# Ecogenomics/CheckM

Hardware: NVIDIA H100
Metric: genomes/hour (higher is better)
Workload: dtype int16 (SSV) / u8 (MSV) / int16 (Viterbi) / f32 (Forward, domain definition)

## Files before the change

checkm_b200/csrc/fwdback_blk.cuh:

```cuda
#pragma once
#include "device_utils.cuh"
#include "engine.hpp"
#include "fwdback.cuh"

namespace ckm {

constexpr int BLK_LOOKAHEAD_MAXQ = 16;

template <int Q, bool TSMEM>
struct BlkModel {
  int M;
  const float *rfb;
  const float4 *tsm;
  float4 t0[TSMEM ? 1 : Q], t1[TSMEM ? 1 : Q];
  int lane;
  __device__ __forceinline__ float4 T0(int q) const { return TSMEM ? tsm[q * 32 + lane] : t0[TSMEM ? 0 : q]; }
  __device__ __forceinline__ float4 T1(int q) const { return TSMEM ? tsm[(Q + q) * 32 + lane] : t1[TSMEM ? 0 : q]; }
};

template <int Q, bool TSMEM>
__device__ __forceinline__ void blk_model_load(BlkModel<Q, TSMEM> &bm, const ModelScalars &ms, const float4 *tfb, const float *rfb,
                                               float4 *tsm, int lane) {
  bm.M = ms.M; bm.lane = lane;
  bm.rfb = rfb + ms.blk_off * 32 * KPAD + lane;
  bm.tsm = tsm;
  const float4 *src = tfb + ms.blk_off * 32 * 2;
  if (TSMEM) {
    __syncwarp();
    for (int q = 0; q < Q; ++q) { tsm[q * 32 + lane] = __ldg(src + (q * 32 + lane) * 2); tsm[(Q + q) * 32 + lane] = __ldg(src + (q * 32 + lane) * 2 + 1); }
    __syncwarp();
  } else {
#pragma unroll
    for (int q = 0; q < Q; ++q) { bm.t0[TSMEM ? 0 : q] = __ldg(src + (q * 32 + lane) * 2); bm.t1[TSMEM ? 0 : q] = __ldg(src + (q * 32 + lane) * 2 + 1); }
  }
}

template <int Q, bool TSMEM, bool FULL, bool STORE_D = true>
__device__ __forceinline__ float forward_blk(const BlkModel<Q, TSMEM> &bm, const uint8_t *__restrict__ res, int L, const Specials sp,
                                             float *xmx, float *full) {
  const int lane = bm.lane;
  float Mx[Q], Ix[Q], Dx[Q];
#pragma unroll
  for (int q = 0; q < Q; ++q) { Mx[q] = 0.0f; Ix[q] = 0.0f; Dx[q] = 0.0f; }
  if (FULL) {
#pragma unroll
    for (int z = 0; z < 3 * Q; ++z) full[z * 32 + lane] = 0.0f;
  }
  float xE = 0.0f, xN = 1.0f, xJ = 0.0f, xB = sp.nmove, xC = 0.0f, totscale = 0.0f;
  if (xmx != nullptr && lane == 0) { xmx[X_E] = xE; xmx[X_N] = xN; xmx[X_J] = xJ; xmx[X_B] = xB; xmx[X_C] = xC; xmx[X_SCALE] = 1.0f; }
  constexpr bool LA = (Q <= BLK_LOOKAHEAD_MAXQ);
  float ecur[Q];
  int xnext;
  if (LA) {
    const float *rp = bm.rfb + (size_t)((L >= 1) ? __ldg(res) : 0) * Q * 32;
#pragma unroll
    for (int q = 0; q < Q; ++q) ecur[q] = __ldg(rp + q * 32);
    xnext = (L >= 2) ? __ldg(res + 1) : 0;
  } else xnext = (L >= 1) ? __ldg(res) : 0;
// ... 209 lines not shown
```

checkm_b200/csrc/kernels_blk.cu:

```cuda
#include "engine.hpp"
#include "device_utils.cuh"
#include "stages.hpp"
#include "fwdback.cuh"
#include "fwdback_blk.cuh"
#include "domdef_common.cuh"

namespace ckm {

constexpr int BLK_WARPS = 4;

template <int Q> __host__ __device__ constexpr size_t blk_tsm_bytes() { return (size_t)Q * 32 * 2 * sizeof(float4); }

template <int Q, bool TSMEM>
__global__ void __launch_bounds__(BLK_WARPS * 32) fwd2_kernel(FilterParams p) {
  extern __shared__ __align__(16) uint8_t bsm[];
  const int lane = threadIdx.x & 31, warp = threadIdx.x >> 5;
  float4 *tsm = reinterpret_cast<float4 *>(bsm) + (size_t)warp * Q * 32 * 2;
  const int n = min(*p.in_count, p.in_cap);
  for (int c = blockIdx.x * BLK_WARPS + warp; c < n; c += gridDim.x * BLK_WARPS) {
    Candidate cd = p.in[c];
    const ModelScalars ms = p.ms[cd.model];
    if (ms.vq != Q) continue;
    const int s = cd.seq, L = p.len[s];
    BlkModel<Q, TSMEM> bm;
    blk_model_load<Q, TSMEM>(bm, ms, p.tfb, p.rfb, tsm, lane);
    const float fsc = forward_blk<Q, TSMEM, false>(bm, p.res + p.off[s], L, make_specials(L, true), nullptr, nullptr);
    cd.fwdsc = fsc;
    const float seq_score = __fdiv_rn(__fsub_rn(fsc, cd.filtersc), 0.69314718055994529f);
    const double P = exp_surv((double)seq_score, (double)ms.evparam[4], (double)ms.evparam[5]);
    cd.P = P;
    if (lane == 0) {
      if (p.dense_fwd != nullptr) p.dense_fwd[(int64_t)p.model_slot[cd.model] * p.nseq + s] = fsc;
      if (P <= p.F3) {
        const int pos = atomicAdd(p.out_count, 1);
        if (pos < p.out_cap) p.out[pos] = cd;
        if (p.dense_passed != nullptr) atomicOr_u8(p.dense_passed, (int64_t)p.model_slot[cd.model] * p.nseq + s, 8);
      }
    }
  }
}

template <int Q, bool TSMEM>
__global__ void __launch_bounds__(BLK_WARPS * 32) regions2_kernel(DomdefParams p) {
  extern __shared__ __align__(16) uint8_t bsm[];
  const int lane = threadIdx.x & 31, warp = threadIdx.x >> 5;
  float4 *tsm = reinterpret_cast<float4 *>(bsm) + (size_t)warp * Q * 32 * 2;
  for (int idx = p.pair_begin + blockIdx.x * BLK_WARPS + warp; idx < p.pair_end; idx += gridDim.x * BLK_WARPS) {
    const int pi = p.pair_order[idx];
    const PairWork pw = p.pairs[pi];
    const ModelScalars ms = p.ms[pw.model];
    if (ms.vq != Q) continue;
    const int L = pw.L;
    BlkModel<Q, TSMEM> bm;
    blk_model_load<Q, TSMEM>(bm, ms, p.tfb, p.rfb, tsm, lane);
    const uint8_t *res = p.res + p.off[pw.seq];
    const Specials sp = make_specials(L, true);
    float *xf = p.xf + pw.row_off * X_NX, *xb = p.xb + pw.row_off * X_NX;
    forward_blk<Q, TSMEM, false>(bm, res, L, sp, xf, nullptr);
    __syncwarp();
    backward_blk<Q, TSMEM, 0>(bm, res, L, sp, xf, xb, nullptr);
    __syncwarp();
    regions_tail(p, pi, L, sp, xf, xb, p.btot + pw.row_off, p.etot + pw.row_off, p.mocc + pw.row_off, p.n2sc + pw.row_off, lane);
    __syncwarp();
  }
}

template <int Q, bool TSMEM>
__global__ void __launch_bounds__(BLK_WARPS * 32) envelope2_kernel(DomdefParams p) {
  extern __shared__ __align__(16) uint8_t bsm[];
  const int lane = threadIdx.x & 31, warp = threadIdx.x >> 5;
  float4 *tsm = reinterpret_cast<float4 *>(bsm) + (size_t)warp * Q * 32 * 2;
  float *null2 = reinterpret_cast<float *>(bsm + (TSMEM ? BLK_WARPS * blk_tsm_bytes<Q>() : 0)) + warp * 32;
  constexpr int QW = Q * 32;
  for (int idx = p.env_begin + blockIdx.x * BLK_WARPS + warp; idx < p.env_end; idx += gridDim.x * BLK_WARPS) {
    const int ei = p.env_order[idx];
    const Envelope env = p.envs[ei];
    const PairWork pw = p.pairs[env.pair];
    const ModelScalars ms = p.ms[pw.model];
    if (ms.vq != Q) continue;
    BlkModel<Q, TSMEM> bm;
    blk_model_load<Q, TSMEM>(bm, ms, p.tfb, p.rfb, tsm, lane);
    const int M = ms.M, Ld = env.j - env.i + 1;
    const uint8_t *res = p.res + p.off[pw.seq] + (env.i - 1);
    const Specials sp = make_specials(pw.L, false);
    const int64_t mat = (int64_t)(Ld + 1) * 3 * QW;
    float *F = p.scratch + env.scratch_off, *Bm = F;
    float *xf = F + mat, *xb = xf + (int64_t)(Ld + 1) * X_NX, *pps = xb + (int64_t)(Ld + 1) * X_NX;
    float *xo = xf;
    float *n2sc = p.n2sc + pw.row_off;
    const float envsc = forward_blk<Q, TSMEM, true, false>(bm, res, Ld, sp, xf, F);
    __syncwarp();
    backward_blk<Q, TSMEM, 2>(bm, res, Ld, sp, xf, xb, F);
    __syncwarp();
    const float scaleproduct = __fdiv_rn(1.0f, xb[X_N]);
    float em[Q], ein[Q];
#pragma unroll
    for (int q = 0; q < Q; ++q) { em[q] = 0.0f; ein[q] = 0.0f; }
    for (int r = 1; r <= Ld; ++r) {
      if (r + 2 <= Ld && lane < Q) {
        const float *fn = F + (int64_t)(r + 2) * 3 * QW;
        prefetch_l2(fn + lane * 32); prefetch_l2(fn + (2 * Q + lane) * 32);
      }
      const float totr = scaleproduct * xf[(int64_t)r * X_NX + X_SCALE];
      const float *fr = F + (int64_t)r * 3 * QW + lane;
      float vm[Q], vi[Q];
#pragma unroll
      for (int q = 0; q < Q; ++q) { vm[q] = fr[q * 32]; vi[q] = fr[(2 * Q + q) * 32]; }
#pragma unroll
      for (int q = 0; q < Q; ++q) {
        const float pm = vm[q] * totr, pi = vi[q] * totr;
        em[q] = (r == 1) ? pm : em[q] + pm;
        ein[q] = (r == 1) ? pi : ein[q] + pi;
      }
    }
// ... 192 lines not shown
          s1 = (t1s * xc[X_N] > t1s * xc[X_J]) ? ST_N : ST_J;
        } else { ok = false; break; }
        if (s1 == ST_M) {
          if (!have_last || s0 == ST_E) { lastMi = i; lastMk = k; have_last = true; }
          firstMi = i; firstMk = k;
          if (p.trace != nullptr && lane == 0) p.trace[pw.row_off + env.i - 1 + i] = k;
        } else if (s1 == ST_I) {
          if (p.trace != nullptr && lane == 0) p.trace[pw.row_off + env.i - 1 + i] = -k;
        }
        if ((s1 == ST_N || s1 == ST_J || s1 == ST_C) && s1 == s0) i--;
        s0 = s1;
      }
      if (!have_last) ok = false;
      hmmfrom = firstMk; hmmto = lastMk; sqfrom = firstMi + env.i - 1; sqto = lastMi + env.i - 1;
    }
#undef CELL
#undef TT0
#undef TT1
    if (lane == 0) {
      DomainOut out;
      out.pair = env.pair; out.ienv = env.i; out.jenv = env.j;
      float domcorrection = 0.0f;
      for (int pos = env.i; pos <= env.j; ++pos) domcorrection += n2sc[pos];
      out.ok = ok ? 1 : 0;
      out.envsc = envsc; out.oasc = oasc; out.domcorrection = domcorrection;
      out.hmmfrom = hmmfrom; out.hmmto = hmmto; out.sqfrom = sqfrom; out.sqto = sqto;
      out.bitscore = 0.f; out.dombias = 0.f; out.pad = 0.f; out.lnP = 0.0;
      p.doms[env.slot] = out;
    }
    __syncwarp();
  }
}

template <int Q, bool TSMEM, class P, class KF>
static int launch_one(KF kern, const P &p, int grid, size_t extra, cudaStream_t st, const char *what) {
  const size_t smem = (TSMEM ? BLK_WARPS * blk_tsm_bytes<Q>() : 0) + extra;
  if (smem > 48 * 1024) {
    cudaError_t e = cudaFuncSetAttribute(kern, cudaFuncAttributeMaxDynamicSharedMemorySize, (int)smem);
    if (e != cudaSuccess) return cuda_fail(e, what);
  }
  kern<<<grid, BLK_WARPS * 32, smem, st>>>(p);
  cudaError_t e = cudaGetLastError();
  return e == cudaSuccess ? CKM_OK : cuda_fail(e, what);
}

#define CKM_CLASS_SWITCH(KERN, EXTRA, WHAT)                                                              \
  switch (cls) {                                                                                        \
    case 0: return launch_one<2, false>(KERN<2, false>, p, grid, EXTRA, st, WHAT);                      \
    case 1: return launch_one<4, false>(KERN<4, false>, p, grid, EXTRA, st, WHAT);                      \
    case 2: return launch_one<6, false>(KERN<6, false>, p, grid, EXTRA, st, WHAT);                      \
    case 3: return launch_one<8, false>(KERN<8, false>, p, grid, EXTRA, st, WHAT);                      \
    case 4: return launch_one<12, true>(KERN<12, true>, p, grid, EXTRA, st, WHAT);                      \
    case 5: return launch_one<16, true>(KERN<16, true>, p, grid, EXTRA, st, WHAT);                      \
    case 6: return launch_one<20, true>(KERN<20, true>, p, grid, EXTRA, st, WHAT);                      \
    case 7: return launch_one<24, true>(KERN<24, true>, p, grid, EXTRA, st, WHAT);                      \
    case 8: return launch_one<28, true>(KERN<28, true>, p, grid, EXTRA, st, WHAT);                      \
    case 9: return launch_one<32, true>(KERN<32, true>, p, grid, EXTRA, st, WHAT);                      \
  }                                                                                                     \
  set_error(WHAT ": bad class"); return CKM_EINVAL;

int launch_fwd2(const FilterParams &p, int cls, int grid, cudaStream_t st) { CKM_CLASS_SWITCH(fwd2_kernel, 0, "fwd2_kernel") }
int launch_regions2(const DomdefParams &p, int cls, int grid, cudaStream_t st) { CKM_CLASS_SWITCH(regions2_kernel, 0, "regions2_kernel") }
int launch_envelopes2(const DomdefParams &p, int cls, int grid, cudaStream_t st) {
  const size_t extra = BLK_WARPS * 32 * sizeof(float);
  CKM_CLASS_SWITCH(envelope2_kernel, extra, "envelope2_kernel")
}

}
```

checkm_b200/csrc/search.cu:

```cuda
#include <algorithm>
#include <atomic>
#include <chrono>
#include <cstdio>
#include <cmath>
#include <cstdlib>
#include <cstring>
#include <memory>
#include <vector>
#include "engine.hpp"
#include "stages.hpp"
#include "pool.hpp"

using namespace ckm;

namespace ckm {

std::atomic<int> g_live_engines{0};
thread_local ckm_engine *g_pool_engine = nullptr;
thread_local int g_pool_next = 0;
constexpr int X_NX_HOST = 6;
struct EnsembleJob;
int ensembles_launch(ckm_engine *e, const ckm_models *m, DomdefParams &p, const std::vector<PairWork> &pairs,
                     const std::vector<Region> &regs, const std::vector<int> &multi_idx, const std::vector<EnsembleCaps> &caps,
                     cudaStream_t st, EnsembleJob **job_out);
int ensembles_collect(EnsembleJob *job, cudaStream_t st, std::vector<std::vector<Envelope>> &out, std::vector<EnsembleCaps> &grow, int *n_over);
void ensembles_abandon(EnsembleJob *job, cudaStream_t st);
enum { CTR_UNIT4 = 0, CTR_UNIT8, CTR_UNIT16, CTR_UNIT32, CTR_CAND, CTR_MSV, CTR_BIAS, CTR_VIT, CTR_FWD, CTR_ENV, CTR_DOM, CTR_VREDO, CTR_SSVRES, CTR_VWORK = 16 , CTR_N = 32 };
enum { EV_SSV = 0, EV_MSV, EV_BIAS, EV_VIT, EV_FWD, EV_CASCADE_END, EV_DOMDEF, EV_END, EV_CALL };

static int64_t env_scratch_budget() {
  if (const char *v = std::getenv("CKM_ENV_SCRATCH_MB")) {
    char *end = nullptr;
    const long long mb = std::strtoll(v, &end, 10);
    if (end != v && *end == '\0' && mb > 0) return (int64_t)std::min<long long>(mb, (long long)1 << 30) * ((int64_t)1 << 20) / (int64_t)sizeof(float);
  }
  size_t free_b = 0, total_b = 0;
  cudaMemGetInfo(&free_b, &total_b);
  const size_t neng = (size_t)std::max(1, g_live_engines.load());
  return (int64_t)std::min<size_t>(total_b * 4 / 10 / neng, (size_t)56 << 30) / (int64_t)sizeof(float);
}
struct SearchKnobs { bool blk, vitp, ssv_resolve, trace; int ens_first; int64_t env_budget; };
static SearchKnobs read_knobs(bool envelopes) {
  auto starts = [](const char *name, char c) { const char *v = std::getenv(name); return v != nullptr && v[0] == c; };
  SearchKnobs k;
  k.blk = !starts("CKM_BLK", '0');
  k.vitp = k.blk && !starts("CKM_VITP", '0');
  k.ssv_resolve = !starts("CKM_SSV_RESOLVE", '0');
  k.trace = starts("CKM_TRACE", '1');
  const char *ens = std::getenv("CKM_ENS_FIRST");
  k.ens_first = ens == nullptr ? -1 : (ens[0] == '0' ? 0 : 1);
  k.env_budget = envelopes ? env_scratch_budget() : 0;
  return k;
}
struct Trace {
  bool on; std::chrono::steady_clock::time_point t0, last;
  explicit Trace(bool on_) : on(on_) { t0 = last = std::chrono::steady_clock::now(); }
  void mark(const char *what) {
    if (!on) return;
    const auto now = std::chrono::steady_clock::now();
    std::fprintf(stderr, "[ckm trace] %-28s +%8.3f ms  (%9.3f)\n", what, std::chrono::duration<double, std::milli>(now - last).count(),
                 std::chrono::duration<double, std::milli>(now - t0).count());
    last = now;
  }
};

static int vq_of(int M) { return (M <= 64) ? 2 : (M <= 128) ? 4 : (M <= 192) ? 6 : (M <= 256) ? 8 : (M <= 384) ? 12 : (M <= 512) ? 16 : (M <= 640) ? 20 : (M <= 768) ? 24 : (M <= 896) ? 28 : (M <= 1024) ? 32 : 0; }
static int cls_of(int M, bool use_blk) {
  if (!use_blk) return N_BLK_CLASSES;
  const int q = vq_of(M);
  for (int c = 0; c < N_BLK_CLASSES; ++c) if (BLK_Q[c] == q) return c;
  return N_BLK_CLASSES;
}

static int fan_out(ckm_engine *e) {
  CKM_CUDA(cudaEventRecord(e->fan_ev, e->stream));
  for (auto &s : e->cls) CKM_CUDA(cudaStreamWaitEvent(s, e->fan_ev, 0));
  return CKM_OK;
}
static int fan_in(ckm_engine *e) {
// ... 1 lines not shown
    CKM_CUDA(cudaEventRecord(e->cls_ev[c], e->cls[c]));
    CKM_CUDA(cudaStreamWaitEvent(e->stream, e->cls_ev[c], 0));
  }
  return CKM_OK;
}

template <class P> static int per_class(ckm_engine *e, const P &p, int (*blocked)(const P &, int, int, cudaStream_t), int blk_per_sm,
                                        int (*unblocked)(const P &, int, cudaStream_t), int per_sm, bool widest_first = false) {
  const int nsm = e->prop.multiProcessorCount;
  int rc;
  if ((rc = fan_out(e))) return rc;
  for (int i = 0; i < ckm_engine::NCLS; ++i) {
    const int c = widest_first ? ckm_engine::NCLS - 1 - i : i;
    if (c == N_BLK_CLASSES) rc = unblocked ? unblocked(p, nsm * per_sm, e->cls[c]) : CKM_OK;
    else rc = p.use_blk ? blocked(p, c, nsm * blk_per_sm, e->cls[c]) : CKM_OK;
    if (rc) return rc;
  }
  return fan_in(e);
}
template <class Launch> static int launch_class_runs(ckm_engine *e, const std::vector<int32_t> &order, const std::vector<int8_t> &cls, size_t b0, size_t b1, Launch launch) {
  const int nsm = e->prop.multiProcessorCount;
  int rc;
  if ((rc = fan_out(e))) return rc;
  while (b0 < b1) {
    size_t r1 = b0; const int c = cls[order[b0]];
    while (r1 < b1 && cls[order[r1]] == c) ++r1;
    const int cnt = (int)(r1 - b0);
    const int grid = c < N_BLK_CLASSES ? std::min(nsm * 8, (cnt + 3) / 4) : std::min(nsm * 4, (cnt + FWD_WARPS - 1) / FWD_WARPS);
    if ((rc = launch(c, (int32_t)b0, (int32_t)r1, grid, e->cls[c]))) return rc;
    e->stats.kernel_launches++;
    b0 = r1;
  }
  return CKM_OK;
}

struct ActiveMasks { DevBuf tile_active, model_active, model_slot; bool all_active = true; };
static FilterParams filter_params(const ckm_models *m, const ckm_seqdb *db, ActiveMasks &am) {
  FilterParams p{};
  p.res = db->d_res; p.off = db->d_off; p.len = db->d_len; p.lenA = db->d_lenA; p.lenB = db->d_lenB; p.tmove_w = db->d_tmove_w;
  p.ms = m->d_scalars; p.bias_eo = m->d_bias_eo; p.rwv = m->d_rwv; p.twv = m->d_twv; p.rfv = m->d_rfv; p.tfv = m->d_tfv;
  p.twb = m->d_twb; p.rwb = m->d_rwb; p.tfb = m->d_tfb; p.rfb = m->d_rfb; p.twp = m->d_twp; p.rwp = m->d_rwp;
  p.row_elems = ((m->maxM + 31) / 32) * 32 + 64;
  p.F1 = 0.02; p.F2 = 1e-3; p.F3 = 1e-5;
  p.model_slot = am.model_slot.as<int32_t>(); p.nseq = db->nseq;
  return p;
}

static DomdefParams domdef_params(const ckm_models *m, const ckm_seqdb *db, const SearchKnobs &k) {
  DomdefParams p{};
  p.res = db->d_res; p.off = db->d_off; p.nullsc = db->d_nullsc; p.ms = m->d_scalars; p.rfv = m->d_rfv; p.tfv = m->d_tfv;
  p.row_elems = ((m->maxM + 31) / 32) * 32 + 64;
  p.tfb = m->d_tfb; p.rfb = m->d_rfb; p.use_blk = k.blk ? 1 : 0;
  return p;
}
static void fill_filter_stats(ckm_engine *e, int64_t n_pairs, const int32_t *ctr, unsigned long long cells, int stages) {
  ckm_stats &s = e->stats;
  s.n_pairs = n_pairs; s.n_cells = (int64_t)cells;
  s.n_ssv_cand = (int64_t)ctr[CTR_CAND] + ctr[CTR_SSVRES]; s.n_msv_exact = ctr[CTR_CAND]; s.n_past_msv = ctr[CTR_MSV]; s.n_past_bias = ctr[CTR_BIAS];
  s.n_past_vit = ctr[CTR_VIT]; s.n_past_fwd = ctr[CTR_FWD]; s.n_vit_redo = ctr[CTR_VREDO];
  float *ms[] = {&s.ms_ssv, &s.ms_msv, &s.ms_bias, &s.ms_vit, &s.ms_fwd};
  for (int i = 0; i < stages; ++i) cudaEventElapsedTime(ms[i], e->ev[EV_SSV + i], e->ev[EV_SSV + i + 1]);
}
static std::vector<float> &logsum_table() {
  static std::vector<float> t = [] {
    std::vector<float> v(16000);
    for (int i = 0; i < 16000; ++i) v[i] = (float)std::log(1.0 + std::exp((double)-i / 1000.0));
    return v;
  }();
  return t;
}

static int build_masks(const ckm_models *m, const ckm_seqdb *db, const int32_t *model_idx, int32_t nmodels,
                       const int64_t *bin_model_offsets, ActiveMasks &am, std::vector<int32_t> &slot_of_model, cudaStream_t st) {
  const int ndb = (int)m->models.size(), nbins = db->nbins, ntiles = (int)m->tiles.size();
  slot_of_model.assign(ndb, -1);
  bool all = (bin_model_offsets == nullptr) && (model_idx == nullptr || nmodels == ndb);
  if (model_idx == nullptr) { for (int i = 0; i < ndb; ++i) slot_of_model[i] = i; }
  else if (bin_model_offsets == nullptr) {
    for (int i = 0; i < nmodels; ++i) {
      if (model_idx[i] < 0 || model_idx[i] >= ndb) { set_error("model index out of range"); return CKM_EINVAL; }
      if (slot_of_model[model_idx[i]] >= 0) { set_error("duplicate model index in query list"); return CKM_EINVAL; }
      slot_of_model[model_idx[i]] = i;
    }
    if (all) for (int i = 0; i < ndb; ++i) if (slot_of_model[i] < 0) all = false;
  }
// ... 150 lines not shown
  if ((rc = launch_bias(p, nsm * 8, st))) return rc;
  CKM_CUDA(cudaEventRecord(e->ev[EV_VIT], st));
  p.in = s2.a.as<Candidate>(); p.in_count = e->d_counters + CTR_BIAS; p.in_cap = s2.cap;
  p.out = s2.b.as<Candidate>(); p.out_count = e->d_counters + CTR_VIT; p.out_cap = s2.cap;
  if ((rc = run_viterbi(e, p, k.vitp))) return rc;
  CKM_CUDA(cudaEventRecord(e->ev[EV_FWD], st));
  p.in = s2.b.as<Candidate>(); p.in_count = e->d_counters + CTR_VIT; p.in_cap = s2.cap;
  p.out = s2.a.as<Candidate>(); p.out_count = e->d_counters + CTR_FWD; p.out_cap = s2.cap;
  if ((rc = per_class(e, p, launch_fwd2, 8, launch_fwd, 4, true))) return rc;
  CKM_CUDA(cudaEventRecord(e->ev[EV_CASCADE_END], st));
  e->stats.kernel_launches += 3 + (k.vitp ? N_BLK_CLASSES : 0) + (p.use_blk ? 2 * N_BLK_CLASSES : 0);
  return CKM_OK;
}

static int64_t envelope_need(const ckm_models *m, const PairWork &pw, const Envelope &en, bool use_blk) {
  const int64_t Ld = en.j - en.i + 1, Mpad = ((m->models[pw.model].M + 1) + 31) / 32 * 32 + 32;
  const int64_t vq = use_blk ? vq_of(m->models[pw.model].M) : 0;
  const int64_t width = vq ? 32 * vq : Mpad;
  return (vq ? 1 : 2) * (Ld + 1) * 3 * width + (Ld + 1) * 15 + 64;
}
static int run_envelope_waves(ckm_engine *e, const ckm_models *m, const std::vector<PairWork> &pairs, DomdefParams &p, int64_t budget,
                              DevBuf &scratch, std::vector<Envelope> &ev, DevBuf &d_ev, DevBuf &d_ord, bool leave_last) {
  if (ev.empty()) return CKM_OK;
  cudaStream_t st = e->stream;
  int rc;
  std::vector<int64_t> need(ev.size());
  std::vector<int8_t> ecls(ev.size());
  for (size_t i = 0; i < ev.size(); ++i) {
    const PairWork &pw = pairs[ev[i].pair];
    need[i] = envelope_need(m, pw, ev[i], p.use_blk != 0);
    ecls[i] = (int8_t)cls_of(m->models[pw.model].M, p.use_blk != 0);
  }
  budget = std::max<int64_t>(budget, *std::max_element(need.begin(), need.end()));
  if ((rc = d_ev.alloc(sizeof(Envelope) * ev.size())) || (rc = d_ord.alloc(sizeof(int32_t) * ev.size()))) return rc;
  std::vector<int32_t> eorder(ev.size());
  for (size_t w0 = 0, w1; w0 < ev.size(); w0 = w1) {
    int64_t tot = 0;
    for (w1 = w0; w1 < ev.size() && (w1 == w0 || tot + need[w1] <= budget); ++w1) { ev[w1].scratch_off = tot; tot += need[w1]; }
    if (sizeof(float) * (size_t)tot > scratch.bytes && (rc = scratch.alloc(sizeof(float) * (size_t)tot))) return rc;
    for (size_t i = w0; i < w1; ++i) eorder[i] = (int32_t)i;
    std::stable_sort(eorder.begin() + w0, eorder.begin() + w1, [&](int32_t a, int32_t b) { return ecls[a] != ecls[b] ? ecls[a] > ecls[b] : need[a] > need[b]; });
    CKM_CUDA(cudaMemcpyAsync(d_ev.as<Envelope>() + w0, ev.data() + w0, sizeof(Envelope) * (w1 - w0), cudaMemcpyHostToDevice, st));
    CKM_CUDA(cudaMemcpyAsync(d_ord.as<int32_t>() + w0, eorder.data() + w0, sizeof(int32_t) * (w1 - w0), cudaMemcpyHostToDevice, st));
    p.envs = d_ev.as<Envelope>(); p.env_order = d_ord.as<int32_t>(); p.scratch = scratch.as<float>();
    if ((rc = launch_class_runs(e, eorder, ecls, w0, w1, [&](int c, int32_t b0, int32_t b1, int grid, cudaStream_t s) -> int {
          p.env_begin = b0; p.env_end = b1; return c < N_BLK_CLASSES ? launch_envelopes2(p, c, grid, s) : launch_envelopes(p, grid, s); }))) return rc;
    CKM_CUDA(cudaStreamSynchronize(st));
    if (w1 < ev.size() || !leave_last) { if ((rc = fan_in(e))) return rc; CKM_CUDA(cudaStreamSynchronize(st)); }
  }
  return CKM_OK;
}

struct QueryPlan { ActiveMasks am; bool per_bin = false; std::vector<std::vector<int32_t>> qorder; int64_t n_pairs = 0; };
static int plan_queries(const ckm_models *m, const ckm_seqdb *db, const int32_t *model_idx, int32_t nmodels, const int64_t *bin_model_offsets, QueryPlan &q, cudaStream_t st) {
  const int ndb = (int)m->models.size();
  if (model_idx == nullptr && bin_model_offsets == nullptr) nmodels = ndb;
  std::vector<int32_t> slot;
  int rc = build_masks(m, db, model_idx, nmodels, bin_model_offsets, q.am, slot, st);
  if (rc) return rc;
  q.per_bin = bin_model_offsets != nullptr;
  if (q.per_bin) {
    q.qorder.assign(db->nbins, std::vector<int32_t>(ndb, -1));
    for (int b = 0; b < db->nbins; ++b) {
      for (int64_t i = bin_model_offsets[b]; i < bin_model_offsets[b + 1]; ++i) q.qorder[b][model_idx[i]] = (int32_t)(i - bin_model_offsets[b]);
      q.n_pairs += (int64_t)db->bin_nseq[b] * (bin_model_offsets[b + 1] - bin_model_offsets[b]);
    }
  } else {
    q.qorder.emplace_back(std::move(slot));
    q.n_pairs = (int64_t)db->nseq * nmodels;
  }
  return CKM_OK;
}

static int run_cascade(ckm_engine *e, const SearchKnobs &k, const ckm_models *m, const ckm_seqdb *db, ActiveMasks &am, int64_t n_pairs, Stage1 &s1, Stage2 &s2, int32_t *ctr) {
  cudaStream_t st = e->stream;
  unsigned long long cells = 0;
  int rc;
  for (int attempt = 0; attempt < QUEUE_ATTEMPTS; ++attempt) {
    if (attempt > 0) e->stats.n_queue_retries++;
// ... 23 lines not shown
    pw.first_dom = 0; pw.ndom_slots = 0; pw.fwdsc = fl[i].fwdsc; pw.filtersc = fl[i].filtersc; pw.usc = fl[i].usc;
    pw.row_off = rows; rows += pw.L + 1;
  }
  return CKM_OK;
}
struct DomainStage {
  DomdefParams p{};
  DevBuf dpairs, dxf, dxb, dvec, dtbl, dregions, dporder, ddoms, dhits, dscratch, denvs, deorder, denvs2, deorder2;
  std::vector<Region> regs;
  std::vector<DomainOut> doms; std::vector<HitOut> hout;
};
static int run_regions(ckm_engine *e, const SearchKnobs &k, const ckm_models *m, const ckm_seqdb *db, const std::vector<PairWork> &pairs, int64_t rows, DomainStage &D, Trace &tr) {
  cudaStream_t st = e->stream;
  const int npairs = (int)pairs.size();
  const size_t rws = (size_t)std::max<int64_t>(rows, 1);
  int rc;
  if ((rc = D.dpairs.alloc(sizeof(PairWork) * pairs.size())) || (rc = D.dxf.alloc(sizeof(float) * rws * X_NX_HOST)) || (rc = D.dxb.alloc(sizeof(float) * rws * X_NX_HOST)) ||
      (rc = D.dvec.alloc(sizeof(float) * rws * 4)) || (rc = D.dtbl.alloc(sizeof(float) * 16000))) return rc;
  const int region_cap = npairs * 8 + 1024;
  if ((rc = D.dregions.alloc(sizeof(Region) * (size_t)region_cap))) return rc;
  CKM_CUDA(cudaMemcpyAsync(D.dpairs.p, pairs.data(), sizeof(PairWork) * pairs.size(), cudaMemcpyHostToDevice, st));
  CKM_CUDA(cudaMemcpyAsync(D.dtbl.p, logsum_table().data(), sizeof(float) * 16000, cudaMemcpyHostToDevice, st));
  CKM_CUDA(cudaMemsetAsync(e->d_counters + CTR_ENV, 0, sizeof(int32_t), st));
  DomdefParams &p = D.p = domdef_params(m, db, k);
  p.pairs = D.dpairs.as<PairWork>(); p.npairs = npairs;
  p.xf = D.dxf.as<float>(); p.xb = D.dxb.as<float>();
  p.btot = D.dvec.as<float>(); p.etot = p.btot + rws; p.mocc = p.etot + rws; p.n2sc = p.mocc + rws;
  p.regions = D.dregions.as<Region>(); p.region_count = e->d_counters + CTR_ENV; p.region_cap = region_cap;
  p.logsum_tbl = D.dtbl.as<float>();
  std::vector<int32_t> order((size_t)npairs);
  std::vector<int8_t> pcls((size_t)npairs);
  for (int i = 0; i < npairs; ++i) { order[i] = i; pcls[i] = (int8_t)cls_of(m->models[pairs[i].model].M, p.use_blk != 0); }
  std::stable_sort(order.begin(), order.end(), [&](int32_t a, int32_t b) { return pcls[a] != pcls[b] ? pcls[a] > pcls[b] : pairs[a].L > pairs[b].L; });
  if ((rc = D.dporder.alloc(sizeof(int32_t) * order.size()))) return rc;
  CKM_CUDA(cudaMemcpyAsync(D.dporder.p, order.data(), sizeof(int32_t) * order.size(), cudaMemcpyHostToDevice, st));
  p.pair_order = D.dporder.as<int32_t>();
  if ((rc = launch_class_runs(e, order, pcls, 0, (size_t)npairs, [&](int c, int32_t b0, int32_t b1, int grid, cudaStream_t s) -> int {
        p.pair_begin = b0; p.pair_end = b1; return c < N_BLK_CLASSES ? launch_regions2(p, c, grid, s) : launch_regions(p, grid, s); }))) return rc;
  if ((rc = fan_in(e))) return rc;
  int32_t nreg = 0;
  CKM_CUDA(cudaMemcpyAsync(&nreg, e->d_counters + CTR_ENV, sizeof(int32_t), cudaMemcpyDeviceToHost, st));
  CKM_CUDA(cudaStreamSynchronize(st));
  tr.mark("regions kernels");
  if (nreg > region_cap) { set_error("region queue overflow"); return CKM_ECAPACITY; }
  D.regs.resize((size_t)nreg);
  if (nreg) CKM_CUDA(cudaMemcpy(D.regs.data(), D.dregions.p, sizeof(Region) * D.regs.size(), cudaMemcpyDeviceToHost));
  std::sort(D.regs.begin(), D.regs.end(), [](const Region &a, const Region &b) { return a.pair != b.pair ? a.pair < b.pair : a.i < b.i; });
  tr.mark("regions sorted");
  return CKM_OK;
}

struct AbandonJob { cudaStream_t st; void operator()(EnsembleJob *job) const { ensembles_abandon(job, st); } };
static int domain_pass(ckm_engine *e, const SearchKnobs &k, const ckm_models *m, std::vector<PairWork> &pairs, DomainStage &D,
                       const std::vector<int> &multi_idx, std::vector<EnsembleCaps> &caps, Trace &tr, bool *grown) {
  cudaStream_t st = e->stream;
  DomdefParams &p = D.p;
  const std::vector<Region> &regs = D.regs; const int nreg = (int)regs.size();
  int rc;
  *grown = false;
  std::vector<int32_t> reg_slot((size_t)nreg);
  std::vector<Envelope> envs1, envs2;
  int32_t nslots = 0;
  for (auto &pw : pairs) { pw.ndom_slots = 0; pw.first_dom = 0; }
  for (int r = 0, mi = 0; r < nreg; ++r) {
    PairWork &pw = pairs[regs[r].pair];
    if (pw.ndom_slots == 0) pw.first_dom = nslots;
    reg_slot[r] = nslots;
    if (!regs[r].multi) { Envelope en{}; en.pair = regs[r].pair; en.i = regs[r].i; en.j = regs[r].j; en.slot = nslots; envs1.push_back(en); }
    const int n = regs[r].multi ? caps[mi++].envelopes : 1;
    nslots += n; pw.ndom_slots += n;
  }
// ... 403 lines not shown
```

checkm_b200/csrc/stages.hpp:

```cpp
#pragma once
#include "engine.hpp"

namespace ckm {

#ifndef CKM_SSV_WARPS
#define CKM_SSV_WARPS 16
#endif
constexpr int SSV_WARPS = CKM_SSV_WARPS;
constexpr int SSV_WARPS_HOST = SSV_WARPS;
constexpr int MSV_WARPS = 8;

struct SsvParams {
  const uint8_t *res; const int64_t *off; const int32_t *len; const int32_t *bin;
  const float *msvB; const int32_t *tjb; const int32_t *order;
  int32_t nseq, seq_chunk, nchunks;
  const TileGroup *groups; const int32_t *group_list; int32_t ngroups;
  const TileDesc *tiles; const TileModel *tile_models;
  const int32_t *chain_first_tile, *chain_ntiles;
  const uint8_t *tile_blob;
  const uint8_t *tile_active;
  const uint8_t *model_active;
  int32_t ntiles, nmodels;
  int32_t *unit_counter;
  int2 *cand; int32_t *cand_count; int32_t cand_cap;
// ... 23 lines not shown
  double F1;
};

int launch_msv_exact(const MsvParams &p, int grid, cudaStream_t stream);
int launch_ssv_bypass(const int32_t *models, int32_t nbypass, int32_t nseq, const int32_t *len, const int32_t *bin,
                      const uint8_t *model_active, int32_t nmodels_db, int2 *cand, int32_t *cand_count, int32_t cand_cap,
                      cudaStream_t stream);
int launch_msv2(const MsvParams &p, int cls, int grid, cudaStream_t stream);

constexpr int VIT_WARPS = 4;
constexpr int FWD_WARPS = 4;
struct FilterParams {
  const uint8_t *res; const int64_t *off; const int32_t *len;
  const float *lenA, *lenB;
  const int16_t *tmove_w;
  const ModelScalars *ms;
  const float *bias_eo; const int16_t *rwv; const int16_t *twv; const float *rfv; const float *tfv;
  const uint4 *twb; const uint32_t *rwb; const float4 *tfb; const float *rfb;
  const uint4 *twp; const uint32_t *rwp;
  Candidate *redo; int32_t *redo_count; int32_t redo_cap;
  int32_t *vit_work;
  const Candidate *in; const int32_t *in_count; int32_t in_cap;
  Candidate *out; int32_t *out_count; int32_t out_cap;
  int32_t row_elems;
  double F1, F2, F3;
  int32_t use_blk;
  float *dense_filtersc, *dense_vit, *dense_fwd; uint8_t *dense_passed;
  const int32_t *model_slot; int32_t nseq;
};
int launch_bias(const FilterParams &p, int grid, cudaStream_t st);
int launch_vit(const FilterParams &p, int grid, cudaStream_t st);
constexpr int N_BLK_CLASSES = 10;
constexpr int BLK_Q[N_BLK_CLASSES] = {2, 4, 6, 8, 12, 16, 20, 24, 28, 32};
int launch_vit2(const FilterParams &p, int cls, int grid, cudaStream_t st);
int launch_vitp(const FilterParams &p, int cls, int grid, cudaStream_t st);
int launch_all_pairs(Candidate *out, int32_t *count, const int32_t *slot_model, int32_t nslots, int32_t nseq, cudaStream_t st);
int launch_fwd(const FilterParams &p, int grid, cudaStream_t st);

#define FLT_MIN_F 1.17549435e-38f
struct PairWork {
  int32_t seq, model, L;
  int32_t first_dom, ndom_slots;
  float   fwdsc, filtersc, usc;
  int64_t row_off;
};
struct Region { int32_t pair, i, j, multi; };
constexpr int ENS_MAXENV = 32;
struct EnsembleCaps { int32_t segments, trace_segments, envelopes; };
constexpr EnsembleCaps ENS_DEFAULT_CAPS = {4096, 64, ENS_MAXENV};
struct Envelope { int32_t pair, i, j, null2_done; int64_t scratch_off; int32_t slot, pad; };
struct DomainOut {
  int32_t pair, ienv, jenv, hmmfrom, hmmto, sqfrom, sqto, ok;
  float   envsc, domcorrection, oasc, bitscore, dombias, pad;
  double  lnP;
};
struct HitOut { float pre_score, score, sum_score; int32_t ndom, valid, pad; double lnP; };
struct DomdefParams {
  const uint8_t *res; const int64_t *off; const float *nullsc;
  const ModelScalars *ms; const float *rfv; const float *tfv;
  const PairWork *pairs; int32_t npairs;
  const int32_t *pair_order; int32_t pair_begin, pair_end;
  float *xf, *xb, *btot, *etot, *mocc, *n2sc;
  int32_t *trace;
  Region *regions; int32_t *region_count; int32_t region_cap;
  const Envelope *envs; const int32_t *env_order; int32_t env_begin, env_end;
  float *scratch;
  DomainOut *doms; HitOut *hits;
  const float *logsum_tbl;
  int32_t row_elems;
  const float4 *tfb; const float *rfb;
  int32_t use_blk;
};
int launch_regions(const DomdefParams &p, int grid, cudaStream_t st);
int launch_envelopes(const DomdefParams &p, int grid, cudaStream_t st);
int launch_scores(const DomdefParams &p, int grid, cudaStream_t st);
int launch_fwd2(const FilterParams &p, int cls, int grid, cudaStream_t st);
int launch_regions2(const DomdefParams &p, int cls, int grid, cudaStream_t st);
int launch_envelopes2(const DomdefParams &p, int cls, int grid, cudaStream_t st);

}
```

Baseline: 33930.

## Share one CTA-wide transition copy across warps working on the same model

For wide model classes (Q>=16), the region and envelope kernels now group work items on the host into chunks of up to four items that share a model. Each CTA fills a single shared-memory transition copy for the chunk, and each warp processes one item against it. This cuts shared memory per CTA by four, which allows more resident blocks, and removes redundant global loads. In exchange it adds __syncthreads per chunk, idle warps when a chunk has fewer than four items, and extra host-side sorting and chunk uploads.

```diff
diff --git a/checkm_b200/csrc/fwdback_blk.cuh b/checkm_b200/csrc/fwdback_blk.cuh
--- a/checkm_b200/csrc/fwdback_blk.cuh
+++ b/checkm_b200/csrc/fwdback_blk.cuh
@@ -19,11 +19,22 @@
 };
 
 template <int Q, bool TSMEM>
-__device__ __forceinline__ void blk_model_load(BlkModel<Q, TSMEM> &bm, const ModelScalars &ms, const float4 *tfb, const float *rfb,
-                                               float4 *tsm, int lane) {
+__device__ __forceinline__ void blk_model_bind(BlkModel<Q, TSMEM> &bm, const ModelScalars &ms, const float *rfb, const float4 *tsm, int lane) {
   bm.M = ms.M; bm.lane = lane;
   bm.rfb = rfb + ms.blk_off * 32 * KPAD + lane;
   bm.tsm = tsm;
+}
+
+template <int Q>
+__device__ __forceinline__ void blk_tsm_fill_cta(float4 *tsm, const ModelScalars &ms, const float4 *tfb) {
+  const float4 *src = tfb + ms.blk_off * 32 * 2;
+  for (int j = threadIdx.x; j < Q * 32; j += blockDim.x) { tsm[j] = __ldg(src + j * 2); tsm[Q * 32 + j] = __ldg(src + j * 2 + 1); }
+}
+
+template <int Q, bool TSMEM>
+__device__ __forceinline__ void blk_model_load(BlkModel<Q, TSMEM> &bm, const ModelScalars &ms, const float4 *tfb, const float *rfb,
+                                               float4 *tsm, int lane) {
+  blk_model_bind(bm, ms, rfb, tsm, lane);
   const float4 *src = tfb + ms.blk_off * 32 * 2;
   if (TSMEM) {
     __syncwarp();
diff --git a/checkm_b200/csrc/kernels_blk.cu b/checkm_b200/csrc/kernels_blk.cu
--- a/checkm_b200/csrc/kernels_blk.cu
+++ b/checkm_b200/csrc/kernels_blk.cu
@@ -8,8 +8,12 @@
 namespace ckm {
 
 constexpr int BLK_WARPS = 4;
+static_assert(BLK_CHUNK == BLK_WARPS, "a chunk of the shared-copy kernels is one item per warp");
 
 template <int Q> __host__ __device__ constexpr size_t blk_tsm_bytes() { return (size_t)Q * 32 * 2 * sizeof(float4); }
+template <int Q, bool TSMEM, bool SHARED> __host__ __device__ constexpr size_t blk_tsm_cta_bytes() {
+  return TSMEM ? (SHARED ? 1 : BLK_WARPS) * blk_tsm_bytes<Q>() : 0;
+}
 
 template <int Q, bool TSMEM>
 __global__ void __launch_bounds__(BLK_WARPS * 32) fwd2_kernel(FilterParams p) {
@@ -40,19 +44,32 @@
   }
 }
 
-template <int Q, bool TSMEM>
+template <int Q, bool TSMEM, bool SHARED>
 __global__ void __launch_bounds__(BLK_WARPS * 32) regions2_kernel(DomdefParams p) {
+  static_assert(TSMEM || !SHARED, "a shared transition copy needs TSMEM");
   extern __shared__ __align__(16) uint8_t bsm[];
   const int lane = threadIdx.x & 31, warp = threadIdx.x >> 5;
-  float4 *tsm = reinterpret_cast<float4 *>(bsm) + (size_t)warp * Q * 32 * 2;
-  for (int idx = p.pair_begin + blockIdx.x * BLK_WARPS + warp; idx < p.pair_end; idx += gridDim.x * BLK_WARPS) {
+  float4 *tsm = reinterpret_cast<float4 *>(bsm) + (SHARED ? 0 : (size_t)warp * Q * 32 * 2);
+  const int begin = SHARED ? p.chunk_begin + blockIdx.x : p.pair_begin + blockIdx.x * BLK_WARPS + warp;
+  const int end = SHARED ? p.chunk_end : p.pair_end, stride = SHARED ? gridDim.x : gridDim.x * BLK_WARPS;
+  for (int it = begin; it < end; it += stride) {
+    int idx = it;
+    if (SHARED) {
+      const int b = p.chunk[it];
+      __syncthreads();
+      blk_tsm_fill_cta<Q>(tsm, p.ms[p.pairs[p.pair_order[b]].model], p.tfb);
+      __syncthreads();
+      idx = b + warp;
+      if (idx >= p.chunk[it + 1]) continue;
+    }
     const int pi = p.pair_order[idx];
     const PairWork pw = p.pairs[pi];
     const ModelScalars ms = p.ms[pw.model];
     if (ms.vq != Q) continue;
     const int L = pw.L;
     BlkModel<Q, TSMEM> bm;
-    blk_model_load<Q, TSMEM>(bm, ms, p.tfb, p.rfb, tsm, lane);
+    if (SHARED) blk_model_bind<Q, TSMEM>(bm, ms, p.rfb, tsm, lane);
+    else blk_model_load<Q, TSMEM>(bm, ms, p.tfb, p.rfb, tsm, lane);
     const uint8_t *res = p.res + p.off[pw.seq];
     const Specials sp = make_specials(L, true);
     float *xf = p.xf + pw.row_off * X_NX, *xb = p.xb + pw.row_off * X_NX;
@@ -65,21 +82,34 @@
   }
 }
 
-template <int Q, bool TSMEM>
+template <int Q, bool TSMEM, bool SHARED>
 __global__ void __launch_bounds__(BLK_WARPS * 32) envelope2_kernel(DomdefParams p) {
+  static_assert(TSMEM || !SHARED, "a shared transition copy needs TSMEM");
   extern __shared__ __align__(16) uint8_t bsm[];
   const int lane = threadIdx.x & 31, warp = threadIdx.x >> 5;
-  float4 *tsm = reinterpret_cast<float4 *>(bsm) + (size_t)warp * Q * 32 * 2;
-  float *null2 = reinterpret_cast<float *>(bsm + (TSMEM ? BLK_WARPS * blk_tsm_bytes<Q>() : 0)) + warp * 32;
+  float4 *tsm = reinterpret_cast<float4 *>(bsm) + (SHARED ? 0 : (size_t)warp * Q * 32 * 2);
+  float *null2 = reinterpret_cast<float *>(bsm + blk_tsm_cta_bytes<Q, TSMEM, SHARED>()) + warp * 32;
   constexpr int QW = Q * 32;
-  for (int idx = p.env_begin + blockIdx.x * BLK_WARPS + warp; idx < p.env_end; idx += gridDim.x * BLK_WARPS) {
+  const int begin = SHARED ? p.chunk_begin + blockIdx.x : p.env_begin + blockIdx.x * BLK_WARPS + warp;
+  const int end = SHARED ? p.chunk_end : p.env_end, stride = SHARED ? gridDim.x : gridDim.x * BLK_WARPS;
+  for (int it = begin; it < end; it += stride) {
+    int idx = it;
+    if (SHARED) {
+      const int b = p.chunk[it];
+      __syncthreads();
+      blk_tsm_fill_cta<Q>(tsm, p.ms[p.pairs[p.envs[p.env_order[b]].pair].model], p.tfb);
+      __syncthreads();
+      idx = b + warp;
+      if (idx >= p.chunk[it + 1]) continue;
+    }
     const int ei = p.env_order[idx];
     const Envelope env = p.envs[ei];
     const PairWork pw = p.pairs[env.pair];
     const ModelScalars ms = p.ms[pw.model];
     if (ms.vq != Q) continue;
     BlkModel<Q, TSMEM> bm;
-    blk_model_load<Q, TSMEM>(bm, ms, p.tfb, p.rfb, tsm, lane);
+    if (SHARED) blk_model_bind<Q, TSMEM>(bm, ms, p.rfb, tsm, lane);
+    else blk_model_load<Q, TSMEM>(bm, ms, p.tfb, p.rfb, tsm, lane);
     const int M = ms.M, Ld = env.j - env.i + 1;
     const uint8_t *res = p.res + p.off[pw.seq] + (env.i - 1);
     const Specials sp = make_specials(pw.L, false);
@@ -338,9 +368,9 @@
   }
 }
 
-template <int Q, bool TSMEM, class P, class KF>
+template <int Q, bool TSMEM, bool SHARED = false, class P, class KF>
 static int launch_one(KF kern, const P &p, int grid, size_t extra, cudaStream_t st, const char *what) {
-  const size_t smem = (TSMEM ? BLK_WARPS * blk_tsm_bytes<Q>() : 0) + extra;
+  const size_t smem = blk_tsm_cta_bytes<Q, TSMEM, SHARED>() + extra;
   if (smem > 48 * 1024) {
     cudaError_t e = cudaFuncSetAttribute(kern, cudaFuncAttributeMaxDynamicSharedMemorySize, (int)smem);
     if (e != cudaSuccess) return cuda_fail(e, what);
@@ -365,11 +395,27 @@
   }                                                                                                     \
   set_error(WHAT ": bad class"); return CKM_EINVAL;
 
+#define CKM_CASE(C, Q_, TS, KERN, EXTRA, WHAT) case C: return launch_one<Q_, TS>(KERN<Q_, TS, false>, p, grid, EXTRA, st, WHAT);
+#define CKM_CASE_WIDE(C, Q_, KERN, EXTRA, WHAT)                                                                         \
+  case C: static_assert(Q_ >= BLK_SHARED_MINQ, "");                                                                    \
+    return shared ? launch_one<Q_, true, true>(KERN<Q_, true, true>, p, grid, EXTRA, st, WHAT)                         \
+                  : launch_one<Q_, true, false>(KERN<Q_, true, false>, p, grid, EXTRA, st, WHAT);
+#define CKM_DOMDEF_CLASS_SWITCH(KERN, EXTRA, WHAT)                                                                      \
+  switch (cls) {                                                                                                       \
+    CKM_CASE(0, 2, false, KERN, EXTRA, WHAT) CKM_CASE(1, 4, false, KERN, EXTRA, WHAT) CKM_CASE(2, 6, false, KERN, EXTRA, WHAT) \
+    CKM_CASE(3, 8, false, KERN, EXTRA, WHAT) CKM_CASE(4, 12, true, KERN, EXTRA, WHAT)                                 \
+    CKM_CASE_WIDE(5, 16, KERN, EXTRA, WHAT) CKM_CASE_WIDE(6, 20, KERN, EXTRA, WHAT) CKM_CASE_WIDE(7, 24, KERN, EXTRA, WHAT) \
+    CKM_CASE_WIDE(8, 28, KERN, EXTRA, WHAT) CKM_CASE_WIDE(9, 32, KERN, EXTRA, WHAT)                                    \
+  }                                                                                                                    \
+  set_error(WHAT ": bad class"); return CKM_EINVAL;
+
 int launch_fwd2(const FilterParams &p, int cls, int grid, cudaStream_t st) { CKM_CLASS_SWITCH(fwd2_kernel, 0, "fwd2_kernel") }
-int launch_regions2(const DomdefParams &p, int cls, int grid, cudaStream_t st) { CKM_CLASS_SWITCH(regions2_kernel, 0, "regions2_kernel") }
-int launch_envelopes2(const DomdefParams &p, int cls, int grid, cudaStream_t st) {
+int launch_regions2(const DomdefParams &p, int cls, bool shared, int grid, cudaStream_t st) {
+  CKM_DOMDEF_CLASS_SWITCH(regions2_kernel, 0, "regions2_kernel")
+}
+int launch_envelopes2(const DomdefParams &p, int cls, bool shared, int grid, cudaStream_t st) {
   const size_t extra = BLK_WARPS * 32 * sizeof(float);
-  CKM_CLASS_SWITCH(envelope2_kernel, extra, "envelope2_kernel")
-}
-
-}
+  CKM_DOMDEF_CLASS_SWITCH(envelope2_kernel, extra, "envelope2_kernel")
+}
+
+}
diff --git a/checkm_b200/csrc/search.cu b/checkm_b200/csrc/search.cu
--- a/checkm_b200/csrc/search.cu
+++ b/checkm_b200/csrc/search.cu
@@ -39,12 +39,13 @@
   const size_t neng = (size_t)std::max(1, g_live_engines.load());
   return (int64_t)std::min<size_t>(total_b * 4 / 10 / neng, (size_t)56 << 30) / (int64_t)sizeof(float);
 }
-struct SearchKnobs { bool blk, vitp, ssv_resolve, trace; int ens_first; int64_t env_budget; };
+struct SearchKnobs { bool blk, vitp, ssv_resolve, trace, blk_shared; int ens_first; int64_t env_budget; };
 static SearchKnobs read_knobs(bool envelopes) {
   auto starts = [](const char *name, char c) { const char *v = std::getenv(name); return v != nullptr && v[0] == c; };
   SearchKnobs k;
   k.blk = !starts("CKM_BLK", '0');
   k.vitp = k.blk && !starts("CKM_VITP", '0');
+  k.blk_shared = k.blk && !starts("CKM_BLK_SHARED", '0');
   k.ssv_resolve = !starts("CKM_SSV_RESOLVE", '0');
   k.trace = starts("CKM_TRACE", '1');
   const char *ens = std::getenv("CKM_ENS_FIRST");
@@ -112,6 +113,37 @@
     b0 = r1;
   }
   return CKM_OK;
+}
+
+static bool cls_shared(const DomdefParams &p, int c) { return p.use_blk && p.blk_shared && c < N_BLK_CLASSES && BLK_Q[c] >= BLK_SHARED_MINQ; }
+template <class ModelOf, class WorkOf>
+static void chunk_by_model(const DomdefParams &p, std::vector<int32_t> &order, const std::vector<int8_t> &cls, size_t b0, size_t b1,
+                           ModelOf model_of, WorkOf work_of, std::vector<int32_t> &chunks) {
+  chunks.clear();
+  std::vector<int32_t> tmp;
+  std::vector<std::pair<size_t, size_t>> runs;
+  for (size_t r0 = b0, r1; r0 < b1; r0 = r1) {
+    const int c = cls[order[r0]];
+    for (r1 = r0; r1 < b1 && cls[order[r1]] == c; ++r1) {}
+    if (!cls_shared(p, c)) { chunks.push_back((int32_t)r0); continue; }
+    std::stable_sort(order.begin() + r0, order.begin() + r1, [&](int32_t a, int32_t b) {
+      return model_of(a) != model_of(b) ? model_of(a) < model_of(b) : work_of(a) > work_of(b); });
+    runs.clear();
+    for (size_t i = r0, j; i < r1; i = j) {
+      for (j = i + 1; j < r1 && j - i < (size_t)BLK_CHUNK && model_of(order[j]) == model_of(order[i]); ++j) {}
+      runs.emplace_back(i, j);
+    }
+    std::stable_sort(runs.begin(), runs.end(), [&](const std::pair<size_t, size_t> &x, const std::pair<size_t, size_t> &y) {
+      return work_of(order[x.first]) > work_of(order[y.first]); });
+    tmp.clear();
+    for (const auto &r : runs) { chunks.push_back((int32_t)(r0 + tmp.size())); tmp.insert(tmp.end(), order.begin() + r.first, order.begin() + r.second); }
+    std::copy(tmp.begin(), tmp.end(), order.begin() + r0);
+  }
+  chunks.push_back((int32_t)b1);
+}
+static void chunk_range(DomdefParams &p, const std::vector<int32_t> &chunks, int32_t b0, int32_t b1) {
+  p.chunk_begin = (int32_t)(std::lower_bound(chunks.begin(), chunks.end(), b0) - chunks.begin());
+  p.chunk_end = (int32_t)(std::lower_bound(chunks.begin(), chunks.end(), b1) - chunks.begin());
 }
 
 struct ActiveMasks { DevBuf tile_active, model_active, model_slot; bool all_active = true; };
@@ -130,7 +162,7 @@
   DomdefParams p{};
   p.res = db->d_res; p.off = db->d_off; p.nullsc = db->d_nullsc; p.ms = m->d_scalars; p.rfv = m->d_rfv; p.tfv = m->d_tfv;
   p.row_elems = ((m->maxM + 31) / 32) * 32 + 64;
-  p.tfb = m->d_tfb; p.rfb = m->d_rfb; p.use_blk = k.blk ? 1 : 0;
+  p.tfb = m->d_tfb; p.rfb = m->d_rfb; p.use_blk = k.blk ? 1 : 0; p.blk_shared = k.blk_shared ? 1 : 0;
   return p;
 }
 static void fill_filter_stats(ckm_engine *e, int64_t n_pairs, const int32_t *ctr, unsigned long long cells, int stages) {
@@ -347,19 +379,26 @@
     ecls[i] = (int8_t)cls_of(m->models[pw.model].M, p.use_blk != 0);
   }
   budget = std::max<int64_t>(budget, *std::max_element(need.begin(), need.end()));
-  if ((rc = d_ev.alloc(sizeof(Envelope) * ev.size())) || (rc = d_ord.alloc(sizeof(int32_t) * ev.size()))) return rc;
-  std::vector<int32_t> eorder(ev.size());
+  if ((rc = d_ev.alloc(sizeof(Envelope) * ev.size())) || (rc = d_ord.alloc(sizeof(int32_t) * (2 * ev.size() + 1)))) return rc;
+  std::vector<int32_t> eorder(ev.size()), chunks;
   for (size_t w0 = 0, w1; w0 < ev.size(); w0 = w1) {
     int64_t tot = 0;
     for (w1 = w0; w1 < ev.size() && (w1 == w0 || tot + need[w1] <= budget); ++w1) { ev[w1].scratch_off = tot; tot += need[w1]; }
     if (sizeof(float) * (size_t)tot > scratch.bytes && (rc = scratch.alloc(sizeof(float) * (size_t)tot))) return rc;
     for (size_t i = w0; i < w1; ++i) eorder[i] = (int32_t)i;
     std::stable_sort(eorder.begin() + w0, eorder.begin() + w1, [&](int32_t a, int32_t b) { return ecls[a] != ecls[b] ? ecls[a] > ecls[b] : need[a] > need[b]; });
+    chunk_by_model(p, eorder, ecls, w0, w1, [&](int32_t a) { return pairs[ev[a].pair].model; }, [&](int32_t a) { return need[a]; }, chunks);
     CKM_CUDA(cudaMemcpyAsync(d_ev.as<Envelope>() + w0, ev.data() + w0, sizeof(Envelope) * (w1 - w0), cudaMemcpyHostToDevice, st));
     CKM_CUDA(cudaMemcpyAsync(d_ord.as<int32_t>() + w0, eorder.data() + w0, sizeof(int32_t) * (w1 - w0), cudaMemcpyHostToDevice, st));
+    CKM_CUDA(cudaMemcpyAsync(d_ord.as<int32_t>() + ev.size() + w0, chunks.data(), sizeof(int32_t) * chunks.size(), cudaMemcpyHostToDevice, st));
     p.envs = d_ev.as<Envelope>(); p.env_order = d_ord.as<int32_t>(); p.scratch = scratch.as<float>();
+    p.chunk = d_ord.as<int32_t>() + ev.size() + w0;
     if ((rc = launch_class_runs(e, eorder, ecls, w0, w1, [&](int c, int32_t b0, int32_t b1, int grid, cudaStream_t s) -> int {
-          p.env_begin = b0; p.env_end = b1; return c < N_BLK_CLASSES ? launch_envelopes2(p, c, grid, s) : launch_envelopes(p, grid, s); }))) return rc;
+          p.env_begin = b0; p.env_end = b1;
+          if (c == N_BLK_CLASSES) return launch_envelopes(p, grid, s);
+          chunk_range(p, chunks, b0, b1);
+          const bool sh = cls_shared(p, c);
+          return launch_envelopes2(p, c, sh, sh ? p.chunk_end - p.chunk_begin : grid, s); }))) return rc;
     CKM_CUDA(cudaStreamSynchronize(st));
     if (w1 < ev.size() || !leave_last) { if ((rc = fan_in(e))) return rc; CKM_CUDA(cudaStreamSynchronize(st)); }
   }
@@ -449,11 +488,19 @@
   std::vector<int8_t> pcls((size_t)npairs);
   for (int i = 0; i < npairs; ++i) { order[i] = i; pcls[i] = (int8_t)cls_of(m->models[pairs[i].model].M, p.use_blk != 0); }
   std::stable_sort(order.begin(), order.end(), [&](int32_t a, int32_t b) { return pcls[a] != pcls[b] ? pcls[a] > pcls[b] : pairs[a].L > pairs[b].L; });
-  if ((rc = D.dporder.alloc(sizeof(int32_t) * order.size()))) return rc;
+  std::vector<int32_t> chunks;
+  chunk_by_model(p, order, pcls, 0, (size_t)npairs, [&](int32_t a) { return pairs[a].model; }, [&](int32_t a) { return pairs[a].L; }, chunks);
+  if ((rc = D.dporder.alloc(sizeof(int32_t) * (order.size() + chunks.size())))) return rc;
   CKM_CUDA(cudaMemcpyAsync(D.dporder.p, order.data(), sizeof(int32_t) * order.size(), cudaMemcpyHostToDevice, st));
+  CKM_CUDA(cudaMemcpyAsync(D.dporder.as<int32_t>() + order.size(), chunks.data(), sizeof(int32_t) * chunks.size(), cudaMemcpyHostToDevice, st));
   p.pair_order = D.dporder.as<int32_t>();
+  p.chunk = p.pair_order + order.size();
   if ((rc = launch_class_runs(e, order, pcls, 0, (size_t)npairs, [&](int c, int32_t b0, int32_t b1, int grid, cudaStream_t s) -> int {
-        p.pair_begin = b0; p.pair_end = b1; return c < N_BLK_CLASSES ? launch_regions2(p, c, grid, s) : launch_regions(p, grid, s); }))) return rc;
+        p.pair_begin = b0; p.pair_end = b1;
+        if (c == N_BLK_CLASSES) return launch_regions(p, grid, s);
+        chunk_range(p, chunks, b0, b1);
+        const bool sh = cls_shared(p, c);
+        return launch_regions2(p, c, sh, sh ? p.chunk_end - p.chunk_begin : grid, s); }))) return rc;
   if ((rc = fan_in(e))) return rc;
   int32_t nreg = 0;
   CKM_CUDA(cudaMemcpyAsync(&nreg, e->d_counters + CTR_ENV, sizeof(int32_t), cudaMemcpyDeviceToHost, st));
diff --git a/checkm_b200/csrc/stages.hpp b/checkm_b200/csrc/stages.hpp
--- a/checkm_b200/csrc/stages.hpp
+++ b/checkm_b200/csrc/stages.hpp
@@ -79,6 +79,8 @@
 int launch_vit(const FilterParams &p, int grid, cudaStream_t st);
 constexpr int N_BLK_CLASSES = 10;
 constexpr int BLK_Q[N_BLK_CLASSES] = {2, 4, 6, 8, 12, 16, 20, 24, 28, 32};
+constexpr int BLK_SHARED_MINQ = 16;
+constexpr int BLK_CHUNK = 4;
 int launch_vit2(const FilterParams &p, int cls, int grid, cudaStream_t st);
 int launch_vitp(const FilterParams &p, int cls, int grid, cudaStream_t st);
 int launch_all_pairs(Candidate *out, int32_t *count, const int32_t *slot_model, int32_t nslots, int32_t nseq, cudaStream_t st);
@@ -111,18 +113,20 @@
   int32_t *trace;
   Region *regions; int32_t *region_count; int32_t region_cap;
   const Envelope *envs; const int32_t *env_order; int32_t env_begin, env_end;
+  const int32_t *chunk; int32_t chunk_begin, chunk_end;
   float *scratch;
   DomainOut *doms; HitOut *hits;
   const float *logsum_tbl;
   int32_t row_elems;
   const float4 *tfb; const float *rfb;
   int32_t use_blk;
+  int32_t blk_shared;
 };
 int launch_regions(const DomdefParams &p, int grid, cudaStream_t st);
 int launch_envelopes(const DomdefParams &p, int grid, cudaStream_t st);
 int launch_scores(const DomdefParams &p, int grid, cudaStream_t st);
 int launch_fwd2(const FilterParams &p, int cls, int grid, cudaStream_t st);
-int launch_regions2(const DomdefParams &p, int cls, int grid, cudaStream_t st);
-int launch_envelopes2(const DomdefParams &p, int cls, int grid, cudaStream_t st);
+int launch_regions2(const DomdefParams &p, int cls, bool shared, int grid, cudaStream_t st);
+int launch_envelopes2(const DomdefParams &p, int cls, bool shared, int grid, cudaStream_t st);
 
 }
```

Result: no change. 34150 (median of 6 runs) (+0.6%).
